# tanushreebanerjee/generative-detection

Measured on AMD Instinct MI355X. Metric: VAE train images/s (fwd+bwd+opt) at 256x256 z=16x16x16, higher is better.
Workload: dtype f32; 1 GPU; autoencoder_kl_16x16x16.yaml, 256x256 synthetic crops, B=32/GPU, rec+KL only (discriminator off, optimizer 0), fp32, VAE phase; global_batch=32, parallelism=dp1

## Files before the change

generative-detection_amd/build.py:

```python
import os
import subprocess
import sys
from concurrent.futures import ThreadPoolExecutor

HERE = os.path.dirname(os.path.abspath(__file__))
CSRC = os.path.join(HERE, "csrc")
OBJ_DIR = os.path.join(HERE, "build")
LIB_PATH = os.path.join(HERE, "libodvae_hip.so")
HIP_SOURCES = ["gemm_f32.hip", "gemm_f32_split.hip", "conv3x3_f32.hip", "conv3x3_wino_f32.hip", "conv3x3_wino4_f32.hip", "conv3x3_wgrad_f32.hip", "conv3x3_wgrad_wino_f32.hip", "groupnorm.hip", "elementwise.hip",
               "gan_f32.hip", "lpips_f32.hip", "patch_u8.hip", "pose_f32.hip", "linear_f32.hip",
               "conv_bf16.hip", "conv_wgrad_bf16.hip", "flash_attn_bf16.hip", "bf16_ops.hip",
               "flash_attn_f32.hip", "linattn_f32.hip", "anomaly.hip"]
CXX_SOURCES = ["runtime.cpp"]
HIPCC = os.environ.get("HIPCC", "/opt/rocm/bin/hipcc")
FLAGS = ["--offload-arch=gfx950", "-O3", "-fPIC", "-std=c++17", "-I", CSRC]
PER_FILE_FLAGS = {"flash_attn_bf16.hip": ["-fno-slp-vectorize"], "gemm_f32_split.hip": ["-fno-slp-vectorize"]}


def _stale(target, deps):
    if not os.path.exists(target):
        return True
    t = os.path.getmtime(target)
    return any(os.path.getmtime(d) > t for d in deps)


def _compile(src):
    obj = os.path.join(OBJ_DIR, os.path.basename(src) + ".o")
    deps = [src, os.path.join(CSRC, "common.h"), os.path.join(CSRC, "bf16_common.h"), os.path.join(CSRC, "gn_finalize.h"), os.path.join(CSRC, "dropout_mask.h"), os.path.join(CSRC, "gemm_f32_tile.h"), os.path.join(CSRC, "resample.h"), os.path.abspath(__file__)]
    if _stale(obj, deps):
        cmd = [HIPCC] + FLAGS + PER_FILE_FLAGS.get(os.path.basename(src), []) + ["-c", src, "-o", obj]
        r = subprocess.run(cmd, capture_output=True, text=True)
        if r.returncode != 0:
# ... 25 lines not shown
```

generative-detection_amd/csrc/gemm_f32.hip:

```cpp
#include "gemm_f32_tile.h"
#include <type_traits>

namespace {

using namespace gemm_tile;
constexpr int LDS_KC = BK + 4;
constexpr int LDS_RC = BM + 4;
constexpr int TILE_FLOATS = BM * LDS_KC;
template <int BKT> struct DmaGeom {
  static constexpr unsigned TILE_B = BM * BKT * 4;
  static constexpr unsigned STAGE_B = 2 * TILE_B;
  static constexpr unsigned LDS_B = 2 * STAGE_B;
  static constexpr int SLOTS = BKT / 4;
  static constexpr int PER_THREAD = BM * SLOTS / 256;
  static constexpr int ROW_SHIFT = BKT == 32 ? 3 : 2, SWZ_SHIFT = BKT == 32 ? 1 : 2, SWZ_MASK = SLOTS - 1;
};
__device__ __forceinline__ float lds_ld32(unsigned a) { return *(const __attribute__((address_space(3))) float*)(uintptr_t)a; }

template <bool KC>
struct TileFetch {
  __amdgpu_buffer_rsrc_t rsrc;
  unsigned voff[4];
  unsigned step_bytes;
  int kvalid;
// ... 360 lines not shown
  const unsigned DMA_LDS_B = lds_bytes;
  const hipError_t e = hipFuncSetAttribute(reinterpret_cast<const void*>(kern), hipFuncAttributeMaxDynamicSharedMemorySize, (int)DMA_LDS_B);
  if (e != hipSuccess) {
    odvae_set_error("gemm_f32: hipFuncSetAttribute failed: %s", hipGetErrorString(e));
    return ODVAE_ERR_HIP;
  }
  hipLaunchKernelGGL(kern, grid, dim3(256), DMA_LDS_B, st, p);
  return ODVAE_OK;
}

}

extern "C" {

int odvae_gemm_select_staging(int mode) {
  const int prev = g_dma_mode;
  g_dma_mode = mode < 0 ? -1 : (mode > 2 ? 2 : mode);
  return prev;
}

size_t odvae_gemm_f32_workspace_bytes(int M, int N, int K, int batch) {
  const int s = choose_splits(M, N, K, batch);
  return s > 1 ? (size_t)s * batch * M * N * sizeof(float) : 0;
}

static int gemm_f32_impl(int transA, int transB, int M, int N, int K, float alpha,
                         const float* A, int lda, int64_t strideA,
                         const float* B, int ldb, int64_t strideB,
                         float* C, int ldc, int64_t strideC,
                         const float* bias, const float* residual, int batch,
                         void* workspace, size_t workspace_bytes, void* stream);

int odvae_gemm_f32(int transA, int transB, int M, int N, int K, float alpha,
                   const float* A, int lda, int64_t strideA,
                   const float* B, int ldb, int64_t strideB,
                   float* C, int ldc, int64_t strideC,
                   const float* bias, const float* residual, int batch,
                   void* workspace, size_t workspace_bytes, void* stream) {
  return gemm_f32_impl(transA, transB, M, N, K, alpha, A, lda, strideA, B, ldb, strideB, C, ldc, strideC, bias, residual, batch,
                       workspace, workspace_bytes, stream);
}

int odvae_gemm_pred_f32(int transA, int transB, int M, int N, int K, float alpha,
                        const float* A, int lda, int64_t strideA,
                        const float* B, int ldb, int64_t strideB,
                        float* C, int ldc, int64_t strideC, int batch, const int* pred, void* stream) {
// ... 203 lines not shown
```

generative-detection_amd/csrc/gemm_f32_split.hip:

```cpp
#include "gemm_f32_tile.h"

namespace {

using namespace gemm_tile;

constexpr unsigned PLANE_B = BM * BK * 2;
constexpr unsigned OPER_B = 3 * PLANE_B;
constexpr unsigned OOB = 0x7FFFFFF0u;
constexpr int HI = 0, MID = 1, LO = 2;

__device__ __forceinline__ unsigned tile_byte(int row, int slot) {
  const int f = ((row >> 2) & 1) | ((((row >> 1) ^ (row >> 3)) & 1) << 1);
  return (unsigned)(row * 64 + ((slot ^ f) << 4));
}

__device__ __forceinline__ void store_unit(unsigned lds_oper, int row, int slot, const float (&x)[8]) {
  u32x4 pl[3];
  split8(x, pl);
  const unsigned a = lds_oper + tile_byte(row, slot);
#pragma unroll
  for (int q = 0; q < 3; ++q) lds_st128(a + q * PLANE_B, pl[q]);
}

template <bool KC>
// ... 43 lines not shown
        }
    } else {
#pragma unroll
      for (int i = 0; i < 2; ++i)
#pragma unroll
        for (int j = 0; j < 8; ++j) {
          const unsigned soff = (unsigned)__builtin_amdgcn_readfirstlane(k0 + 16 * i + j) * ld_bytes;
          unsigned vo = voff[0];
          if (tail && k0 + 8 * (tid >> 7) + 16 * i + j >= kvalid) vo = OOB;
          x[i][j] = __uint_as_float(__builtin_amdgcn_raw_buffer_load_b32(rsrc, vo, soff, 0));
        }
    }
  }
  __device__ __forceinline__ void store(unsigned lds_oper) const {
    const int tid = threadIdx.x;
#pragma unroll
    for (int i = 0; i < 2; ++i) {
      if (KC) store_unit(lds_oper, (tid + 256 * i) >> 2, tid & 3, x[i]);
      else    store_unit(lds_oper, tid & 127, (tid >> 7) + 2 * i, x[i]);
    }
  }
};

template <bool A_KC, bool B_KC, int EPI>
__global__ __launch_bounds__(256, 3) void gemm_f32_split_kernel(GemmParams p) {
  constexpr bool ROWNORM = EPI == EPI_ROWNORM, EXPB = EPI == EPI_EXPB, SMB = EPI == EPI_SMB;
  static_assert(!ROWNORM || A_KC, "the row sums are taken by the k-contiguous loader");
  static_assert(!(EXPB || SMB) || (A_KC && B_KC), "the T x T tails belong to the NT form");
  __shared__ __attribute__((aligned(16))) char smem[2 * OPER_B];
  const int tile_m = blockIdx.x % p.tiles_m, tile_n = blockIdx.x / p.tiles_m, batch = blockIdx.z;
  const int m0 = tile_m * BM, n0 = tile_n * BN;
  const float* A = p.A + batch * p.sA;
  const float* B = p.B + batch * p.sB;
  const int lane = threadIdx.x & 63, wave = threadIdx.x >> 6;
  const int wm = wave >> 1, wn = wave & 1, li = lane & 31, h = lane >> 5;

  TileOut out;
  out.init(p.M, p.N, p.ldc, m0, n0);

  f32x16 acc[2][2];
#pragma unroll
  for (int a = 0; a < 2; ++a)
#pragma unroll
    for (int b = 0; b < 2; ++b)
#pragma unroll
      for (int r = 0; r < 16; ++r) acc[a][b][r] = 0.f;

  const unsigned ldsA = lds_addr_of(smem), ldsB = ldsA + OPER_B;
  unsigned adrA[2], adrB[2];
#pragma unroll
  for (int kk = 0; kk < 2; ++kk) {
    adrA[kk] = ldsA + tile_byte(wm * 64 + li, 2 * kk + h);
    adrB[kk] = ldsB + tile_byte(wn * 64 + li, 2 * kk + h);
  }

  SplitLoader<A_KC> fa;
  SplitLoader<B_KC> fb;
  fa.init(A, p.lda, m0, p.M, p.K);
  fb.init(B, p.ldb, n0, p.N, p.K);
  float rowl[2] = {0.f, 0.f};
  auto stage = [&]() {
    if constexpr (ROWNORM) {
#pragma unroll
      for (int i = 0; i < 2; ++i)
        rowl[i] += ((fa.x[i][0] + fa.x[i][1]) + (fa.x[i][2] + fa.x[i][3])) + ((fa.x[i][4] + fa.x[i][5]) + (fa.x[i][6] + fa.x[i][7]));
    }
    fa.store(ldsA);
    fb.store(ldsB);
  };
  auto products = [&]() {
#pragma unroll
    for (int kk = 0; kk < 2; ++kk) {
      bf16x8 a[2][3], b[2][3];
#pragma unroll
      for (int t = 0; t < 2; ++t)
#pragma unroll
        for (int q = 0; q < 3; ++q) {
          a[t][q] = frag_from_u32x4(lds_ld128(adrA[kk] + t * 2048u + q * PLANE_B));
          b[t][q] = frag_from_u32x4(lds_ld128(adrB[kk] + t * 2048u + q * PLANE_B));
        }
      constexpr int ORDER[6][2] = {{LO, HI}, {HI, LO}, {MID, MID}, {MID, HI}, {HI, MID}, {HI, HI}};
#pragma unroll
// ... 67 lines not shown

namespace gemm_tile {

bool split_eligible(int staging_mode, int transB, int M, int N, int K, int batch, const float* bias, const float* residual) {
  return staging_mode == -1 && choose_splits(M, N, K, batch) == 1 && transB == 0 && K >= 1024 && !bias && !residual;
}

constexpr int SPLIT_TT_MIN_K = 64;
bool split_tt_eligible(int staging_mode, int M, int N, int K, int batch) {
  return staging_mode == -1 && (int64_t)ceil_div(M, BM) * ceil_div(N, BN) * batch >= 512 && K >= SPLIT_TT_MIN_K;
}

int launch_split(const GemmParams& p, int transA, int epi, int batch, hipStream_t st) {
  const dim3 grid(p.tiles_m * ceil_div(p.N, BN), 1, batch), block(256);
  if (epi == EPI_EXPB)          hipLaunchKernelGGL((gemm_f32_split_kernel<true, true, EPI_EXPB>), grid, block, 0, st, p);
  else if (epi == EPI_SMB)      hipLaunchKernelGGL((gemm_f32_split_kernel<true, true, EPI_SMB>), grid, block, 0, st, p);
  else if (epi == EPI_ROWNORM)  hipLaunchKernelGGL((gemm_f32_split_kernel<true, false, EPI_ROWNORM>), grid, block, 0, st, p);
  else if (!transA)             hipLaunchKernelGGL((gemm_f32_split_kernel<true, false, EPI_NONE>), grid, block, 0, st, p);
  else                          hipLaunchKernelGGL((gemm_f32_split_kernel<false, false, EPI_NONE>), grid, block, 0, st, p);
  ODVAE_LAUNCH_CHECK("gemm_f32 (bf16 split)");
  return ODVAE_OK;
}

}
```

generative-detection_amd/csrc/gemm_f32_tile.h:

```cpp
#pragma once
#include "bf16_common.h"

namespace gemm_tile {

constexpr int BM = 128, BN = 128, BK = 32;

struct GemmParams {
  const float* A; const float* B; float* C;
  const float* bias; const float* residual;
  float* partial;
  int M, N, K;
  int lda, ldb, ldc;
  int64_t sA, sB, sC;
  float alpha;
  int splits, k_per_split;
  int tiles_m;
  const float* rowsub; const float* emul; int64_t sRow;
  const float* rowmul;
  float* rowout; int* flag;
  const int* pred;
};
constexpr int EPI_NONE = 0, EPI_SMB = 1, EPI_EXPB = 2, EPI_ROWNORM = 3;

inline int choose_splits(int M, int N, int K, int batch) {
// ... 99 lines not shown
  }

#define GEMM_TILE_STORE_SMB(o, crsrc, ersrc, acc, alpha, rmv)                                                                            \
  {                                                                                                                                      \
    _Pragma("unroll") for (int mt_ = 0; mt_ < 2; ++mt_) {                                                                                \
      float pv_[2][16];                                                                                                                  \
      _Pragma("unroll") for (int r_ = 0; r_ < 16; ++r_) {                                                                                \
        const unsigned rb_ = (o).row_byte(mt_, r_);                                                                                      \
        _Pragma("unroll") for (int nt_ = 0; nt_ < 2; ++nt_)                                                                              \
          pv_[nt_][r_] = __uint_as_float(__builtin_amdgcn_raw_buffer_load_b32(ersrc, rb_ + (o).colbyte[nt_], 0, 0));                     \
      }                                                                                                                                  \
      _Pragma("unroll") for (int r_ = 0; r_ < 16; ++r_) {                                                                                \
        const unsigned rb_ = (o).row_byte(mt_, r_);                                                                                      \
        _Pragma("unroll") for (int nt_ = 0; nt_ < 2; ++nt_)                                                                              \
          __builtin_amdgcn_raw_buffer_store_b32(__float_as_uint((acc)[mt_][nt_][r_] * ((alpha) * (rmv)[mt_][r_]) * pv_[nt_][r_]), crsrc, \
                                                rb_ + (o).colbyte[nt_], 0, 0);                                                           \
      }                                                                                                                                  \
    }                                                                                                                                    \
  }

bool split_eligible(int staging_mode, int transB, int M, int N, int K, int batch, const float* bias, const float* residual);
bool split_tt_eligible(int staging_mode, int M, int N, int K, int batch);
int launch_split(const GemmParams& p, int transA, int epi, int batch, hipStream_t st);

}
```

generative-detection_amd/lib.py:

```python
import ctypes
import os
import re

import torch

_HERE = os.path.dirname(os.path.abspath(__file__))
LIB_PATH = os.path.join(_HERE, "libodvae_hip.so")
HEADER_PATH = os.path.join(os.path.dirname(_HERE), "include", "odvae_hip.h")

_c = ctypes
_P, _I, _L, _F, _Z = _c.c_void_p, _c.c_int, _c.c_int64, _c.c_float, _c.c_size_t
_D, _U64 = _c.c_double, _c.c_uint64

ABI_VERSION = 4

PROTOTYPES = {
    "odvae_last_error": (_c.c_char_p, []),
    "odvae_abi_version": (_I, []),
    "odvae_target_arch": (_c.c_char_p, []),
    "odvae_gemm_f32_workspace_bytes": (_Z, [_I, _I, _I, _I]),
    "odvae_gemm_select_staging": (_I, [_I]),
    "odvae_gemm_f32": (_I, [_I, _I, _I, _I, _I, _F, _P, _I, _L, _P, _I, _L, _P, _I, _L, _P, _P, _I, _P, _Z, _P]),
    "odvae_gemm_softmax_bwd_f32": (_I, [_I, _I, _I, _F, _P, _I, _L, _P, _I, _L, _P, _P, _L, _P, _I, _L, _I, _P]),
    "odvae_rowdot_f32": (_I, [_P, _P, _L, _I, _P, _P]),
    "odvae_attn_row_bound_f32": (_I, [_P, _I, _I, _I, _P, _P, _P, _P]),
    "odvae_gemm_exp_bound_f32": (_I, [_I, _I, _I, _F, _P, _I, _L, _P, _I, _L, _P, _L, _P, _I, _L, _I, _P]),
    "odvae_gemm_rownorm_f32": (_I, [_I, _I, _I, _P, _I, _L, _P, _I, _L, _P, _I, _L, _P, _L, _P, _I, _P]),
    "odvae_gemm_pred_f32": (_I, [_I, _I, _I, _I, _I, _F, _P, _I, _L, _P, _I, _L, _P, _I, _L, _I, _P, _P]),
    "odvae_softmax_rows_pred_f32": (_I, [_P, _P, _L, _I, _F, _P, _P, _P]),
    "odvae_rowdot_scale_f32": (_I, [_P, _P, _P, _L, _I, _P, _P, _P]),
    "odvae_gemm_softmax_bwd_scaled_f32": (_I, [_I, _I, _I, _F, _P, _I, _L, _P, _I, _L, _P, _P, _P, _L, _P, _I, _L, _I, _P]),
    "odvae_conv3x3_pack_reduce_pad": (_I, [_I]),
    "odvae_conv3x3_pack_out_pad": (_I, [_I]),
    "odvae_conv3x3_pack_floats": (_Z, [_I, _I]),
    "odvae_conv3x3_pack_f32": (_I, [_P, _I, _I, _P, _P, _P]),
    "odvae_conv3x3_up_pack_floats": (_Z, [_I, _I]),
    "odvae_conv3x3_pack_up_f32": (_I, [_P, _I, _I, _P, _P, _P]),
    "odvae_conv3x3_wino_reduce_pad": (_I, [_I]),
    "odvae_conv3x3_wino_out_pad": (_I, [_I]),
    "odvae_conv3x3_wino_pack_floats": (_Z, [_I, _I]),
    "odvae_conv3x3_pack_wino_f32": (_I, [_P, _I, _I, _P, _P, _P]),
    "odvae_conv3x3_wino_f32": (_I, [_P, _I, _I, _I, _I, _P, _I, _P, _P, _P, _I, _P]),
    "odvae_conv3x3_wino4_reduce_pad": (_I, [_I]),
    "odvae_conv3x3_wino4_out_pad": (_I, [_I]),
    "odvae_conv3x3_wino4_pack_floats": (_Z, [_I, _I]),
    "odvae_conv3x3_wino4_supported": (_I, [_I, _I, _I, _I]),
    "odvae_conv3x3_pack_wino4_f32": (_I, [_P, _I, _I, _P, _P, _P]),
    "odvae_conv3x3_pack_wino_batch": (_I, [_P, _I, _P]),
    "odvae_conv3x3_pack_wino4_batch": (_I, [_P, _I, _P]),
    "odvae_conv3x3_wino4_f32": (_I, [_P, _I, _I, _I, _I, _P, _I, _P, _P, _P, _I, _P]),
    "odvae_conv3x3_wino4_stats_chunks": (_I, [_I, _I]),
    "odvae_conv3x3_wino4_stats_f32": (_I, [_P, _I, _I, _I, _I, _P, _I, _P, _P, _P, _P, _I, _P]),
    "odvae_conv3x3_wino4_up_f32": (_I, [_P, _I, _I, _I, _I, _P, _I, _P, _P, _P, _P, _I, _P]),
    "odvae_conv3x3_wino4_pool_f32": (_I, [_P, _I, _I, _I, _I, _P, _I, _P, _P]),
# ... 245 lines not shown
```

generative-detection_amd/ops.py:

```python
import collections
import contextlib
import os
import weakref

import torch
from torch.autograd import Function

from . import lib as _lib

CL = torch.channels_last


def _L():
    return _lib.load()


BF16 = torch.bfloat16


def _cl(t, dtype=torch.float32):
    _lib.require_device(t, dtypes=(dtype,))
    if t.dim() != 4:
        raise ValueError("expected a 4-d NCHW tensor, got shape %s" % (tuple(t.shape),))
    n, c, h, w = t.shape
# ... 545 lines not shown
        if ctx.needs_input_grad[1]:
            dw2 = torch.empty(cout, cin, dtype=torch.float32, device=x.device)
            gemm(1, 0, cout, cin, m, 1.0, dy, cout, 0, x, cin, 0, dw2, cin, 0)
            dw = dw2.view(cout, cin, 1, 1)
        if ctx.has_bias and ctx.needs_input_grad[2]:
            db = _colsum(dy, m, cout)
        dres = dy if ctx.has_res and ctx.needs_input_grad[3] else None
        return dx, dw, db, dres


def conv1x1(x, weight, bias=None, residual=None, out_f32=False):
    if x.dtype == BF16:
        return _ConvB.apply(x, weight, bias, residual, 4, bool(out_f32))
    return _Conv1x1.apply(x, weight, bias, residual)


FUSED_SOFTMAX_BWD = os.environ.get("ODVAE_ATTN_UNFUSED", "0") != "1"


ATTN_FOLDED_SOFTMAX = os.environ.get("ODVAE_ATTN_FOLDED_SOFTMAX", "1") != "0"
_ATTN_LAST_FLAG = None


def _qkv_views(t, c):
    off = t.storage_offset()
    return tuple(t.as_strided((1,), (1,), off + i * c) for i in range(3))


class _Attention(Function):

    @staticmethod
    def forward(ctx, qkv):
        L = _L()
        qkv = _cl(qkv)
        n, c3, h, w = qkv.shape
        c = c3 // 3
        t = h * w
        scale = float(c) ** -0.5
        p = torch.empty(n, t, t, dtype=torch.float32, device=qkv.device)
        o = _new_cl(n, c, h, w, qkv)
        q, k, v = _qkv_views(qkv, c)
        sq = t * c3
        rinv = None
        if ATTN_FOLDED_SOFTMAX and L.odvae_gemm_f32_workspace_bytes(t, t, c, n) == 0 and L.odvae_gemm_f32_workspace_bytes(t, c, t, n) == 0:
            st = _lib.stream_ptr()
            bound = torch.empty(2, n * t, dtype=torch.float32, device=qkv.device)
            rinv = torch.empty(n * t, dtype=torch.float32, device=qkv.device)
            flag = torch.empty(1, dtype=torch.int32, device=qkv.device)
            _lib.check(L.odvae_attn_row_bound_f32(q.data_ptr(), n, t, c, bound.data_ptr(), bound[1].data_ptr(), flag.data_ptr(), st), "attn_row_bound")
            tag = KERNEL_EVENTS.begin(secondary=True)
            _lib.check(L.odvae_gemm_exp_bound_f32(t, t, c, scale, q.data_ptr(), c3, sq, k.data_ptr(), c3, sq, bound.data_ptr(), t,
                                                  p.data_ptr(), t, t * t, n, st), "gemm_exp_bound")
            KERNEL_EVENTS.end("gemm_f32", 2.0 * t * t * c * n, tag, 4.0 * n * (2 * t * c + t * t))
            tag = KERNEL_EVENTS.begin(secondary=True)
            _lib.check(L.odvae_gemm_rownorm_f32(t, c, t, p.data_ptr(), t, t * t, v.data_ptr(), c3, sq, o.data_ptr(), c, t * c,
                                                rinv.data_ptr(), t, flag.data_ptr(), n, st), "gemm_rownorm")
            KERNEL_EVENTS.end("gemm_f32", 2.0 * t * t * c * n, tag, 4.0 * n * (2 * t * c + t * t))
            _lib.check(L.odvae_gemm_pred_f32(0, 1, t, t, c, 1.0, q.data_ptr(), c3, sq, k.data_ptr(), c3, sq, p.data_ptr(), t, t * t, n,
                                             flag.data_ptr(), st), "gemm_pred(QK^T)")
            _lib.check(L.odvae_softmax_rows_pred_f32(p.data_ptr(), p.data_ptr(), n * t, t, scale, flag.data_ptr(), rinv.data_ptr(), st), "softmax_rows_pred")
            _lib.check(L.odvae_gemm_pred_f32(0, 0, t, c, t, 1.0, p.data_ptr(), t, t * t, v.data_ptr(), c3, sq, o.data_ptr(), c, t * c, n,
                                             flag.data_ptr(), st), "gemm_pred(PV)")
            global _ATTN_LAST_FLAG
            _ATTN_LAST_FLAG = flag
        else:
            gemm(0, 1, t, t, c, 1.0, q, c3, sq, k, c3, sq, p, t, t * t, batch=n)
            _lib.check(L.odvae_softmax_rows_f32(p.data_ptr(), p.data_ptr(), n * t, t, scale, _lib.stream_ptr()), "softmax_rows")
            gemm(0, 0, t, c, t, 1.0, p, t, t * t, v, c3, sq, o, c, t * c, batch=n)
        ctx.folded = rinv is not None
        if rinv is not None:
            ctx.save_for_backward(qkv, p, o, rinv)
        else:
            ctx.save_for_backward(qkv, p, o)
        return o

    @staticmethod
    def backward(ctx, do):
        L = _L()
        if ctx.folded:
            qkv, p, o, rinv = ctx.saved_tensors
        else:
            (qkv, p, o), rinv = ctx.saved_tensors, None
        do = _cl(do)
        n, c3, h, w = qkv.shape
        c = c3 // 3
        t = h * w
        scale = float(c) ** -0.5
        sq = t * c3
        q, k, v = _qkv_views(qkv, c)
        dqkv = _new_cl(n, c3, h, w, qkv)
        dq, dk, dv = _qkv_views(dqkv, c)
        if rinv is not None:
            drow = torch.empty(n * t, dtype=torch.float32, device=p.device)
            dos = torch.empty_like(do)
            _lib.check(L.odvae_rowdot_scale_f32(do.data_ptr(), o.data_ptr(), rinv.data_ptr(), n * t, c, drow.data_ptr(), dos.data_ptr(),
                                                _lib.stream_ptr()), "rowdot_scale")
            gemm(1, 0, t, c, t, 1.0, p, t, t * t, dos, c, t * c, dv, c3, sq, batch=n)
            del dos
            dp = torch.empty_like(p)
            tag = KERNEL_EVENTS.begin(secondary=True)
            _lib.check(L.odvae_gemm_softmax_bwd_scaled_f32(t, t, c, scale, do.data_ptr(), c, t * c, v.data_ptr(), c3, sq, p.data_ptr(),
                                                           drow.data_ptr(), rinv.data_ptr(), t, dp.data_ptr(), t, t * t, n, _lib.stream_ptr()),
                       "gemm_softmax_bwd_scaled")
            KERNEL_EVENTS.end("gemm_f32", 2.0 * t * t * c * n, tag, 4.0 * n * (2 * t * c + 2 * t * t))
            gemm(0, 0, t, c, t, 1.0, dp, t, t * t, k, c3, sq, dq, c3, sq, batch=n)
            gemm(1, 0, t, c, t, 1.0, dp, t, t * t, q, c3, sq, dk, c3, sq, batch=n)
            return dqkv
        gemm(1, 0, t, c, t, 1.0, p, t, t * t, do, c, t * c, dv, c3, sq, batch=n)
        dp = torch.empty_like(p)
        if FUSED_SOFTMAX_BWD:
            drow = torch.empty(n * t, dtype=torch.float32, device=p.device)
            _lib.check(L.odvae_rowdot_f32(do.data_ptr(), o.data_ptr(), n * t, c, drow.data_ptr(), _lib.stream_ptr()), "rowdot")
            tag = KERNEL_EVENTS.begin(secondary=True)
            _lib.check(L.odvae_gemm_softmax_bwd_f32(t, t, c, scale, do.data_ptr(), c, t * c, v.data_ptr(), c3, sq, p.data_ptr(),
                                                    drow.data_ptr(), t, dp.data_ptr(), t, t * t, n, _lib.stream_ptr()),
                       "gemm_softmax_bwd")
            KERNEL_EVENTS.end("gemm_f32", 2.0 * t * t * c * n, tag, 4.0 * n * (2 * t * c + 2 * t * t))
        else:
            gemm(0, 1, t, t, c, 1.0, do, c, t * c, v, c3, sq, dp, t, t * t, batch=n)
            _lib.check(L.odvae_softmax_rows_bwd_f32(p.data_ptr(), dp.data_ptr(), dp.data_ptr(), n * t, t, scale,
                                                    _lib.stream_ptr()), "softmax_rows_bwd")
        gemm(0, 0, t, c, t, 1.0, dp, t, t * t, k, c3, sq, dq, c3, sq, batch=n)
        gemm(1, 0, t, c, t, 1.0, dp, t, t * t, q, c3, sq, dk, c3, sq, batch=n)
        return dqkv


ATTN_SCORE_BUDGET = int(float(os.environ.get("ODVAE_ATTN_SCORE_BUDGET_GB", "4")) * 2 ** 30)


# ... 1302 lines not shown
```

include/odvae_hip.h:

```cpp
#ifndef ODVAE_HIP_H
#define ODVAE_HIP_H

#include <stddef.h>
#include <stdint.h>

#ifdef __cplusplus
extern "C" {
#endif

#define ODVAE_ABI_VERSION 4
#define ODVAE_OK 0
#define ODVAE_ERR_ARG 1
#define ODVAE_ERR_WORKSPACE 2
#define ODVAE_ERR_HIP 3

const char* odvae_last_error(void);
int odvae_abi_version(void);
const char* odvae_target_arch(void);

size_t odvae_gemm_f32_workspace_bytes(int M, int N, int K, int batch);
int odvae_gemm_select_staging(int mode);
int odvae_gemm_f32(int transA, int transB, int M, int N, int K, float alpha,
                   const float* A, int lda, int64_t strideA,
                   const float* B, int ldb, int64_t strideB,
// ... 85 lines not shown
int odvae_groupnorm_fused_timeouts(void);
int odvae_device_health(int* gn_timeouts, int* attn_fallbacks, int inject_gn_timeouts, int inject_attn_fallbacks);
int odvae_attn_softmax_fallbacks(int add);
int odvae_groupnorm_recentred(int add);

int odvae_softmax_rows_f32(const float* x, float* y, int64_t rows, int cols, float scale, void* stream);
int odvae_softmax_rows_bwd_f32(const float* p, const float* dp, float* ds, int64_t rows, int cols, float scale, void* stream);
int odvae_rowdot_f32(const float* a, const float* b, int64_t rows, int cols, float* out, void* stream);
int odvae_gemm_softmax_bwd_f32(int M, int N, int K, float alpha, const float* A, int lda, int64_t strideA,
                               const float* B, int ldb, int64_t strideB, const float* P, const float* rowdot,
                               int64_t strideRow, float* dS, int ldc, int64_t strideC, int batch, void* stream);
int odvae_attn_row_bound_f32(const float* qkv, int N, int T, int C, float* bound, float* nk_scratch, int* flag, void* stream);
int odvae_gemm_exp_bound_f32(int M, int N, int K, float alpha, const float* A, int lda, int64_t strideA, const float* B, int ldb, int64_t strideB,
                             const float* rowbound, int64_t strideRow, float* E, int ldc, int64_t strideC, int batch, void* stream);
int odvae_gemm_rownorm_f32(int M, int N, int K, const float* A, int lda, int64_t strideA, const float* B, int ldb, int64_t strideB,
                           float* C, int ldc, int64_t strideC, float* rinv, int64_t strideRow, int* flag, int batch, void* stream);
int odvae_gemm_pred_f32(int transA, int transB, int M, int N, int K, float alpha, const float* A, int lda, int64_t strideA,
                        const float* B, int ldb, int64_t strideB, float* C, int ldc, int64_t strideC, int batch, const int* pred, void* stream);
int odvae_softmax_rows_pred_f32(const float* x, float* y, int64_t rows, int cols, float scale, const int* pred, float* ones, void* stream);
int odvae_rowdot_scale_f32(const float* a, const float* b, const float* row_scale, int64_t rows, int cols, float* out, float* a_scaled, void* stream);
int odvae_gemm_softmax_bwd_scaled_f32(int M, int N, int K, float alpha, const float* A, int lda, int64_t strideA,
                                      const float* B, int ldb, int64_t strideB, const float* E, const float* rowdot, const float* rinv,
                                      int64_t strideRow, float* dS, int ldc, int64_t strideC, int batch, void* stream);
int odvae_upsample2x_bwd_f32(const float* du, float* dx, int N, int H, int W, int C, void* stream);
int odvae_avgpool2x2_f32(const float* x, float* y, int N, int H, int W, int C, float* gn_partial, int gn_groups, int chunks, void* stream);
int odvae_avgpool2x2_bwd_f32(const float* dy, float* dx, int N, int H, int W, int C, void* stream);
int odvae_upsample2x_f32(const float* x, float* u, int N, int H, int W, int C, float* gn_partial, int gn_groups, int chunks, void* stream);
int odvae_tanh_f32(const float* x, float* y, int64_t n, void* stream);
int odvae_tanh_bwd_f32(const float* y, const float* dy, float* dx, int64_t n, void* stream);
int odvae_rescale_minmax_f32(const float* x_nchw, float* y_nhwc, int N, int C, int HW, float* minmax_out,
                             void* workspace, size_t workspace_bytes, void* stream);
int odvae_gaussian_sample_f32(const float* moments, const float* eps, float* z, int N, int HW, int Cz, void* stream);
int odvae_gaussian_kl_f32(const float* moments, float* kl, int N, int HW, int Cz, void* stream);
int odvae_gaussian_bwd_f32(const float* moments, const float* eps, const float* dz, const float* dkl,
                           float* dmoments, int N, int HW, int Cz, void* stream);
int odvae_l1_masked_sum_f32(const float* x, const float* xr, const float* mask, float* out, int N, int HW, int C,
                            void* workspace, size_t workspace_bytes, void* stream);
int odvae_l1_masked_bwd_f32(const float* x, const float* xr, const float* mask, const float* g, float* dxr,
                            int N, int HW, int C, void* stream);
size_t odvae_colsum_workspace_bytes(int64_t rows, int C);
int odvae_colsum_f32(const float* x, int64_t rows, int C, float* out, void* workspace, size_t workspace_bytes, void* stream);
int odvae_grad_norm_f32(const float* g, int64_t n, float max_norm, float* out, void* workspace, size_t workspace_bytes, void* stream);
int odvae_adam_step_f32(float* p, const float* g, float* m, float* v, int64_t n, float lr, float beta1, float beta2,
                        float eps, int step, const float* clip, void* stream);
int odvae_grad_accumulate_segments_per_launch(void);
int odvae_grad_accumulate_f32(float* arena, int64_t arena_numel, const int64_t* dst_off, const float* const* src, const int64_t* numel,
// ... 122 lines not shown
```

Measured before the change: 154.9 images/s.

## Pre-split attention GEMM operands into bf16 planes once and reuse across GEMMs

Adds a presplit kernel that converts f32 operands (Q, K, V, dO, optionally row-scaled) into three bf16 planes stored in global memory. The split-bf16 GEMM kernel gets a plane loader that reads these planes with b128 buffer loads instead of splitting f32 values per tile. Attention forward and backward use this path when the shapes are eligible. Splitting happens once per operand instead of once per tile per GEMM, at the cost of extra plane buffers and extra presplit launches.

```diff
diff --git a/generative-detection_amd/build.py b/generative-detection_amd/build.py
--- a/generative-detection_amd/build.py
+++ b/generative-detection_amd/build.py
@@ -7,7 +7,7 @@
 CSRC = os.path.join(HERE, "csrc")
 OBJ_DIR = os.path.join(HERE, "build")
 LIB_PATH = os.path.join(HERE, "libodvae_hip.so")
-HIP_SOURCES = ["gemm_f32.hip", "gemm_f32_split.hip", "conv3x3_f32.hip", "conv3x3_wino_f32.hip", "conv3x3_wino4_f32.hip", "conv3x3_wgrad_f32.hip", "conv3x3_wgrad_wino_f32.hip", "groupnorm.hip", "elementwise.hip",
+HIP_SOURCES = ["gemm_f32.hip", "gemm_f32_split.hip", "gemm_presplit.hip", "conv3x3_f32.hip", "conv3x3_wino_f32.hip", "conv3x3_wino4_f32.hip", "conv3x3_wgrad_f32.hip", "conv3x3_wgrad_wino_f32.hip", "groupnorm.hip", "elementwise.hip",
                "gan_f32.hip", "lpips_f32.hip", "patch_u8.hip", "pose_f32.hip", "linear_f32.hip",
                "conv_bf16.hip", "conv_wgrad_bf16.hip", "flash_attn_bf16.hip", "bf16_ops.hip",
                "flash_attn_f32.hip", "linattn_f32.hip", "anomaly.hip"]
diff --git a/generative-detection_amd/csrc/gemm_f32.hip b/generative-detection_amd/csrc/gemm_f32.hip
--- a/generative-detection_amd/csrc/gemm_f32.hip
+++ b/generative-detection_amd/csrc/gemm_f32.hip
@@ -406,6 +406,10 @@
 size_t odvae_gemm_f32_workspace_bytes(int M, int N, int K, int batch) {
   const int s = choose_splits(M, N, K, batch);
   return s > 1 ? (size_t)s * batch * M * N * sizeof(float) : 0;
+}
+
+int odvae_gemm_split_eligible(int nt, int M, int N, int K, int batch) {
+  return nt ? split_tt_eligible(g_dma_mode, M, N, K, batch) : split_eligible(g_dma_mode, 0, M, N, K, batch, nullptr, nullptr);
 }
 
 static int gemm_f32_impl(int transA, int transB, int M, int N, int K, float alpha,
diff --git a/generative-detection_amd/csrc/gemm_f32_split.hip b/generative-detection_amd/csrc/gemm_f32_split.hip
--- a/generative-detection_amd/csrc/gemm_f32_split.hip
+++ b/generative-detection_amd/csrc/gemm_f32_split.hip
@@ -1,4 +1,5 @@
 #include "gemm_f32_tile.h"
+#include <type_traits>
 
 namespace {
 
@@ -89,16 +90,60 @@
   }
 };
 
-template <bool A_KC, bool B_KC, int EPI>
+struct PlaneLoader {
+  __amdgpu_buffer_rsrc_t rsrc;
+  unsigned voff[2];
+  unsigned plane_bytes;
+  int kvalid;
+  u32x4 v[2][3];
+
+  __device__ __forceinline__ void init(const bf16_t* G, int ld, int64_t plane_stride, int row0, int nrows, int K) {
+    const int tid = threadIdx.x;
+    kvalid = K;
+    plane_bytes = (unsigned)plane_stride * 2u;
+    const int rows = min(BM, nrows - row0);
+    const int64_t bytes = (2 * plane_stride + (int64_t)(rows - 1) * ld + ((K + 7) & ~7)) * 2;
+    rsrc = __builtin_amdgcn_make_buffer_rsrc(const_cast<bf16_t*>(G) + (int64_t)row0 * ld, 0, (int)(bytes < 0x7FFFFFF0ll ? bytes : 0x7FFFFFF0ll), 0x00020000);
+#pragma unroll
+    for (int i = 0; i < 2; ++i) {
+      const int u = tid + 256 * i;
+      voff[i] = (u >> 2) < rows ? (unsigned)(((u >> 2) * ld + 8 * (u & 3)) * 2) : OOB;
+    }
+  }
+  template <bool TAIL>
+  __device__ __forceinline__ void load(int k0) {
+    const int tid = threadIdx.x;
+    const bool tail = TAIL && k0 + BK > kvalid;
+    const unsigned soff = (unsigned)__builtin_amdgcn_readfirstlane(k0) * 2u;
+#pragma unroll
+    for (int i = 0; i < 2; ++i) {
+      unsigned vo = voff[i];
+      if (tail && k0 + 8 * (tid & 3) >= kvalid) vo = OOB;
+#pragma unroll
+      for (int q = 0; q < 3; ++q) v[i][q] = __builtin_amdgcn_raw_buffer_load_b128(rsrc, vo, soff + (unsigned)q * plane_bytes, 0);
+    }
+  }
+  __device__ __forceinline__ void store(unsigned lds_oper) const {
+    const int tid = threadIdx.x;
+#pragma unroll
+    for (int i = 0; i < 2; ++i) {
+      const unsigned a = lds_oper + tile_byte((tid + 256 * i) >> 2, tid & 3);
+#pragma unroll
+      for (int q = 0; q < 3; ++q) lds_st128(a + q * PLANE_B, v[i][q]);
+    }
+  }
+};
+
+template <bool A_KC, bool B_KC, int EPI, bool A_PL = false, bool B_PL = false>
 __global__ __launch_bounds__(256, 3) void gemm_f32_split_kernel(GemmParams p) {
   constexpr bool ROWNORM = EPI == EPI_ROWNORM, EXPB = EPI == EPI_EXPB, SMB = EPI == EPI_SMB;
-  static_assert(!ROWNORM || A_KC, "the row sums are taken by the k-contiguous loader");
+  static_assert(!ROWNORM || (A_KC && !A_PL), "the row sums are taken by the k-contiguous loader, from the unsplit values");
   static_assert(!(EXPB || SMB) || (A_KC && B_KC), "the T x T tails belong to the NT form");
   __shared__ __attribute__((aligned(16))) char smem[2 * OPER_B];
   const int tile_m = blockIdx.x % p.tiles_m, tile_n = blockIdx.x / p.tiles_m, batch = blockIdx.z;
   const int m0 = tile_m * BM, n0 = tile_n * BN;
-  const float* A = p.A + batch * p.sA;
-  const float* B = p.B + batch * p.sB;
+  [[maybe_unused]] const float* A = p.A + batch * p.sA;
+  [[maybe_unused]] const float* B = p.B + batch * p.sB;
   const int lane = threadIdx.x & 63, wave = threadIdx.x >> 6;
   const int wm = wave >> 1, wn = wave & 1, li = lane & 31, h = lane >> 5;
 
@@ -121,10 +166,12 @@
     adrB[kk] = ldsB + tile_byte(wn * 64 + li, 2 * kk + h);
   }
 
-  SplitLoader<A_KC> fa;
-  SplitLoader<B_KC> fb;
-  fa.init(A, p.lda, m0, p.M, p.K);
-  fb.init(B, p.ldb, n0, p.N, p.K);
+  std::conditional_t<A_PL, PlaneLoader, SplitLoader<A_KC>> fa;
+  std::conditional_t<B_PL, PlaneLoader, SplitLoader<B_KC>> fb;
+  if constexpr (A_PL) fa.init(reinterpret_cast<const bf16_t*>(p.A) + 3 * batch * p.sA, p.lda, p.sA, m0, p.M, p.K);
+  else                fa.init(A, p.lda, m0, p.M, p.K);
+  if constexpr (B_PL) fb.init(reinterpret_cast<const bf16_t*>(p.B) + 3 * batch * p.sB, p.ldb, p.sB, n0, p.N, p.K);
+  else                fb.init(B, p.ldb, n0, p.N, p.K);
   float rowl[2] = {0.f, 0.f};
   auto stage = [&]() {
     if constexpr (ROWNORM) {
@@ -238,4 +285,15 @@
   return ODVAE_OK;
 }
 
-}
+int launch_split_planes(const GemmParams& p, int transA, int epi, int batch, hipStream_t st) {
+  const dim3 grid(p.tiles_m * ceil_div(p.N, BN), 1, batch), block(256);
+  if (epi == EPI_EXPB)          hipLaunchKernelGGL((gemm_f32_split_kernel<true, true, EPI_EXPB, true, true>), grid, block, 0, st, p);
+  else if (epi == EPI_SMB)      hipLaunchKernelGGL((gemm_f32_split_kernel<true, true, EPI_SMB, true, true>), grid, block, 0, st, p);
+  else if (epi == EPI_ROWNORM)  hipLaunchKernelGGL((gemm_f32_split_kernel<true, false, EPI_ROWNORM, false, true>), grid, block, 0, st, p);
+  else if (!transA)             hipLaunchKernelGGL((gemm_f32_split_kernel<true, false, EPI_NONE, false, true>), grid, block, 0, st, p);
+  else                          hipLaunchKernelGGL((gemm_f32_split_kernel<false, false, EPI_NONE, false, true>), grid, block, 0, st, p);
+  ODVAE_LAUNCH_CHECK("gemm_f32 (bf16 split, pre-split operands)");
+  return ODVAE_OK;
+}
+
+}
diff --git a/generative-detection_amd/csrc/gemm_f32_tile.h b/generative-detection_amd/csrc/gemm_f32_tile.h
--- a/generative-detection_amd/csrc/gemm_f32_tile.h
+++ b/generative-detection_amd/csrc/gemm_f32_tile.h
@@ -145,5 +145,6 @@
 bool split_eligible(int staging_mode, int transB, int M, int N, int K, int batch, const float* bias, const float* residual);
 bool split_tt_eligible(int staging_mode, int M, int N, int K, int batch);
 int launch_split(const GemmParams& p, int transA, int epi, int batch, hipStream_t st);
+int launch_split_planes(const GemmParams& p, int transA, int epi, int batch, hipStream_t st);
 
 }
diff --git a/generative-detection_amd/csrc/gemm_presplit.hip b/generative-detection_amd/csrc/gemm_presplit.hip
--- /dev/null
+++ b/generative-detection_amd/csrc/gemm_presplit.hip
@@ -0,0 +1,176 @@
+#include "gemm_f32_tile.h"
+
+namespace {
+
+using namespace gemm_tile;
+
+__device__ __forceinline__ f32x4 ld_f32x4(const float* p) { return *reinterpret_cast<const f32x4*>(p); }
+
+__global__ __launch_bounds__(256) void presplit_channel_kernel(const float* __restrict__ x, int ld, int64_t sx, const float* __restrict__ rs,
+                                                               int T, int C, int Cp, bf16_t* __restrict__ out) {
+  const int upr = Cp >> 3, n = blockIdx.y;
+  const int64_t units = (int64_t)T * upr;
+  for (int64_t u = (int64_t)blockIdx.x * 256 + threadIdx.x; u < units; u += (int64_t)gridDim.x * 256) {
+    const int tok = (int)(u / upr), c0 = (int)(u - (int64_t)tok * upr) * 8;
+    const float* px = x + n * sx + (int64_t)tok * ld + c0;
+    const f32x4 a = ld_f32x4(px);
+    const f32x4 b = c0 + 4 < C ? ld_f32x4(px + 4) : f32x4{0.f, 0.f, 0.f, 0.f};
+    float v[8] = {a.x, a.y, a.z, a.w, b.x, b.y, b.z, b.w};
+    if (rs) {
+      const float r = rs[(int64_t)n * T + tok];
+#pragma unroll
+      for (int j = 0; j < 8; ++j) v[j] = __fmul_rn(v[j], r);
+    }
+    u32x4 pl[3];
+    split8(v, pl);
+#pragma unroll
+    for (int q = 0; q < 3; ++q)
+      *reinterpret_cast<u32x4*>(out + (((int64_t)n * 3 + q) * T + tok) * Cp + c0) = pl[q];
+  }
+}
+
+constexpr int PT = 64, PC = 64;
+__global__ __launch_bounds__(256) void presplit_token_kernel(const float* __restrict__ x, int ld, int64_t sx, const float* __restrict__ rs,
+                                                             int T, int C, int Tp, bf16_t* __restrict__ out) {
+  __shared__ float tile[PT][PC + 1];
+  const int t0 = blockIdx.x * PT, c0 = blockIdx.y * PC, n = blockIdx.z, tid = threadIdx.x;
+#pragma unroll
+  for (int i = 0; i < 4; ++i) {
+    const int f = tid + 256 * i, tok = f >> 4, c4 = (f & 15) * 4;
+    f32x4 a = {0.f, 0.f, 0.f, 0.f};
+    if (t0 + tok < T && c0 + c4 < C) {
+      a = ld_f32x4(x + n * sx + (int64_t)(t0 + tok) * ld + c0 + c4);
+      if (rs) {
+        const float r = rs[(int64_t)n * T + t0 + tok];
+        a.x = __fmul_rn(a.x, r); a.y = __fmul_rn(a.y, r); a.z = __fmul_rn(a.z, r); a.w = __fmul_rn(a.w, r);
+      }
+    }
+    tile[tok][c4] = a.x; tile[tok][c4 + 1] = a.y; tile[tok][c4 + 2] = a.z; tile[tok][c4 + 3] = a.w;
+  }
+  __syncthreads();
+#pragma unroll
+  for (int i = 0; i < 2; ++i) {
+    const int u = tid + 256 * i, tu = u & 7, ch = u >> 3;
+    float v[8];
+#pragma unroll
+    for (int j = 0; j < 8; ++j) v[j] = tile[tu * 8 + j][ch];
+    u32x4 pl[3];
+    split8(v, pl);
+    if (c0 + ch < C && t0 + tu * 8 < Tp) {
+#pragma unroll
+      for (int q = 0; q < 3; ++q)
+        *reinterpret_cast<u32x4*>(out + (((int64_t)n * 3 + q) * C + c0 + ch) * Tp + t0 + tu * 8) = pl[q];
+    }
+  }
+}
+
+inline int round8(int v) { return (v + 7) & ~7; }
+
+int check_planes(const char* who, const void* P, int ld, int64_t ps, int64_t stride, int rows, int K) {
+  ODVAE_CHECK_ARG(P && ((uintptr_t)P & 15) == 0, "%s: planes must be non-null and 16-byte aligned", who);
+  ODVAE_CHECK_ARG(ld % 8 == 0 && ps % 8 == 0 && stride % 8 == 0, "%s: plane ld / plane stride / batch stride must be multiples of 8 (ld=%d)", who, ld);
+  ODVAE_CHECK_ARG(ld >= round8(K), "%s: plane ld %d < K rounded up to 8 (K=%d)", who, ld, K);
+  ODVAE_CHECK_ARG(ps >= (int64_t)rows * ld, "%s: plane stride %lld < rows * ld", who, (long long)ps);
+  ODVAE_CHECK_ARG(stride == 3 * ps, "%s: the three planes of an image are adjacent: batch stride %lld != 3 * plane stride %lld", who,
+                  (long long)stride, (long long)ps);
+  ODVAE_CHECK_ARG((2 * ps + (int64_t)BM * ld) * 2 < 0x7FFFFFF0ll, "%s: one block's window over the three planes exceeds 2 GiB", who);
+  return ODVAE_OK;
+}
+
+void base_params(GemmParams& p, int M, int N, int K, float alpha, float* C, int ldc, int64_t strideC) {
+  p.C = C; p.bias = nullptr; p.residual = nullptr; p.partial = nullptr;
+  p.M = M; p.N = N; p.K = K; p.ldc = ldc; p.sC = strideC; p.alpha = alpha;
+  p.splits = 1; p.k_per_split = ceil_div(K, BK) * BK; p.tiles_m = ceil_div(M, BM);
+  p.rowsub = nullptr; p.emul = nullptr; p.sRow = 0; p.rowmul = nullptr; p.rowout = nullptr; p.flag = nullptr; p.pred = nullptr;
+}
+
+int tdeep_impl(const char* who, int transA, int epi, GemmParams& p, const float* A, int lda, int64_t strideA,
+               const void* Bp, int ldbp, int64_t psB, int64_t strideBp, int batch, void* stream) {
+  ODVAE_CHECK_ARG(p.M > 0 && p.N > 0 && p.K > 0 && batch > 0 && batch <= 65535, "%s: bad shape M=%d N=%d K=%d batch=%d", who, p.M, p.N, p.K, batch);
+  ODVAE_CHECK_ARG(A && p.C, "%s: null operand", who);
+  ODVAE_CHECK_ARG((int64_t)BM * p.ldc * 4 < 0x7FFFFFF0ll, "%s: ldc %d too large for 32-bit tile offsets", who, p.ldc);
+  ODVAE_CHECK_ARG(lda % 4 == 0 && strideA % 4 == 0 && ((uintptr_t)A & 15) == 0, "%s: lda / strideA must be multiples of 4 floats, A 16-byte aligned", who);
+  if (!transA) ODVAE_CHECK_ARG(p.K % 4 == 0, "%s: a k-contiguous A needs K %% 4 == 0 (K=%d)", who, p.K);
+  ODVAE_CHECK_ARG((transA ? (int64_t)p.k_per_split * lda : (int64_t)BM * lda) * 4 < 0x7FFFFFF0ll, "%s: one block's window of A exceeds 2 GiB", who);
+  const int rc = check_planes(who, Bp, ldbp, psB, strideBp, p.N, p.K);
+  if (rc != ODVAE_OK) return rc;
+  p.A = A; p.lda = lda; p.sA = strideA;
+  p.B = static_cast<const float*>(Bp); p.ldb = ldbp; p.sB = psB;
+  return launch_split_planes(p, transA, epi, batch, static_cast<hipStream_t>(stream));
+}
+
+int nt_impl(const char* who, int epi, GemmParams& p, const void* Ap, int ldap, int64_t psA, int64_t strideAp,
+            const void* Bp, int ldbp, int64_t psB, int64_t strideBp, int batch, void* stream) {
+  ODVAE_CHECK_ARG(p.M > 0 && p.N > 0 && p.K > 0 && batch > 0 && batch <= 65535, "%s: bad shape M=%d N=%d K=%d batch=%d", who, p.M, p.N, p.K, batch);
+  ODVAE_CHECK_ARG(p.C && p.rowsub, "%s: null operand", who);
+  ODVAE_CHECK_ARG((int64_t)BM * p.ldc * 4 < 0x7FFFFFF0ll, "%s: ldc %d too large for 32-bit tile offsets", who, p.ldc);
+  int rc = check_planes(who, Ap, ldap, psA, strideAp, p.M, p.K);
+  if (rc != ODVAE_OK) return rc;
+  rc = check_planes(who, Bp, ldbp, psB, strideBp, p.N, p.K);
+  if (rc != ODVAE_OK) return rc;
+  p.A = static_cast<const float*>(Ap); p.lda = ldap; p.sA = psA;
+  p.B = static_cast<const float*>(Bp); p.ldb = ldbp; p.sB = psB;
+  return launch_split_planes(p, 0, epi, batch, static_cast<hipStream_t>(stream));
+}
+
+}
+
+extern "C" {
+
+int odvae_split_planes_f32(const float* x, int ld, int64_t stride, const float* row_scale, int batch, int T, int C, int token_contiguous,
+                           void* planes, void* stream) {
+  ODVAE_CHECK_ARG(x && planes && batch > 0 && batch <= 65535 && T > 0 && C > 0, "split_planes: bad arguments (batch=%d T=%d C=%d)", batch, T, C);
+  ODVAE_CHECK_ARG(C % 4 == 0 && ld % 4 == 0 && ld >= C && stride % 4 == 0, "split_planes: C, ld and the batch stride must be multiples of 4 floats, ld >= C");
+  ODVAE_CHECK_ARG(((uintptr_t)x & 15) == 0 && ((uintptr_t)planes & 15) == 0, "split_planes: x and planes must be 16-byte aligned");
+  hipStream_t st = static_cast<hipStream_t>(stream);
+  bf16_t* out = static_cast<bf16_t*>(planes);
+  if (token_contiguous) {
+    ODVAE_CHECK_ARG(ceil_div(C, PC) <= 65535, "split_planes: C %d too large", C);
+    hipLaunchKernelGGL(presplit_token_kernel, dim3(ceil_div(T, PT), ceil_div(C, PC), batch), dim3(256), 0, st, x, ld, stride, row_scale, T, C, round8(T), out);
+  } else {
+    const int Cp = round8(C);
+    const int64_t blocks = ceil_div64((int64_t)T * (Cp >> 3), 256);
+    hipLaunchKernelGGL(presplit_channel_kernel, dim3((unsigned)std::min<int64_t>(blocks, 65536), batch), dim3(256), 0, st, x, ld, stride, row_scale, T, C, Cp, out);
+  }
+  ODVAE_LAUNCH_CHECK("split_planes");
+  return ODVAE_OK;
+}
+
+int odvae_gemm_presplit_f32(int transA, int M, int N, int K, float alpha, const float* A, int lda, int64_t strideA,
+                            const void* Bp, int ldbp, int64_t planeB, int64_t strideBp, float* C, int ldc, int64_t strideC, int batch, void* stream) {
+  GemmParams p;
+  base_params(p, M, N, K, alpha, C, ldc, strideC);
+  if (transA) ODVAE_CHECK_ARG(M % 4 == 0, "gemm_presplit: transA needs M %% 4 == 0 (M=%d)", M);
+  return tdeep_impl("gemm_presplit", transA != 0, EPI_NONE, p, A, lda, strideA, Bp, ldbp, planeB, strideBp, batch, stream);
+}
+
+int odvae_gemm_rownorm_presplit_f32(int M, int N, int K, const float* A, int lda, int64_t strideA, const void* Bp, int ldbp, int64_t planeB,
+                                    int64_t strideBp, float* C, int ldc, int64_t strideC, float* rinv, int64_t strideRow, int* flag, int batch,
+                                    void* stream) {
+  ODVAE_CHECK_ARG(rinv, "gemm_rownorm_presplit: null operand");
+  GemmParams p;
+  base_params(p, M, N, K, 1.f, C, ldc, strideC);
+  p.sRow = strideRow; p.rowout = rinv; p.flag = flag;
+  return tdeep_impl("gemm_rownorm_presplit", 0, EPI_ROWNORM, p, A, lda, strideA, Bp, ldbp, planeB, strideBp, batch, stream);
+}
+
+int odvae_gemm_exp_bound_presplit_f32(int M, int N, int K, float alpha, const void* Ap, int ldap, int64_t planeA, int64_t strideAp,
+                                      const void* Bp, int ldbp, int64_t planeB, int64_t strideBp, const float* rowbound, int64_t strideRow,
+                                      float* E, int ldc, int64_t strideC, int batch, void* stream) {
+  GemmParams p;
+  base_params(p, M, N, K, alpha, E, ldc, strideC);
+  p.rowsub = rowbound; p.sRow = strideRow;
+  return nt_impl("gemm_exp_bound_presplit", EPI_EXPB, p, Ap, ldap, planeA, strideAp, Bp, ldbp, planeB, strideBp, batch, stream);
+}
+
+int odvae_gemm_softmax_bwd_presplit_f32(int M, int N, int K, float alpha, const void* Ap, int ldap, int64_t planeA, int64_t strideAp,
+                                        const void* Bp, int ldbp, int64_t planeB, int64_t strideBp, const float* P, const float* rowdot,
+                                        const float* rinv, int64_t strideRow, float* dS, int ldc, int64_t strideC, int batch, void* stream) {
+  ODVAE_CHECK_ARG(P, "gemm_softmax_bwd_presplit: null operand");
+  GemmParams p;
+  base_params(p, M, N, K, alpha, dS, ldc, strideC);
+  p.rowsub = rowdot; p.emul = P; p.sRow = strideRow; p.rowmul = rinv;
+  return nt_impl("gemm_softmax_bwd_presplit", EPI_SMB, p, Ap, ldap, planeA, strideAp, Bp, ldbp, planeB, strideBp, batch, stream);
+}
+
+}
diff --git a/generative-detection_amd/lib.py b/generative-detection_amd/lib.py
--- a/generative-detection_amd/lib.py
+++ b/generative-detection_amd/lib.py
@@ -30,6 +30,12 @@
     "odvae_softmax_rows_pred_f32": (_I, [_P, _P, _L, _I, _F, _P, _P, _P]),
     "odvae_rowdot_scale_f32": (_I, [_P, _P, _P, _L, _I, _P, _P, _P]),
     "odvae_gemm_softmax_bwd_scaled_f32": (_I, [_I, _I, _I, _F, _P, _I, _L, _P, _I, _L, _P, _P, _P, _L, _P, _I, _L, _I, _P]),
+    "odvae_gemm_split_eligible": (_I, [_I, _I, _I, _I, _I]),
+    "odvae_split_planes_f32": (_I, [_P, _I, _L, _P, _I, _I, _I, _I, _P, _P]),
+    "odvae_gemm_presplit_f32": (_I, [_I, _I, _I, _I, _F, _P, _I, _L, _P, _I, _L, _L, _P, _I, _L, _I, _P]),
+    "odvae_gemm_rownorm_presplit_f32": (_I, [_I, _I, _I, _P, _I, _L, _P, _I, _L, _L, _P, _I, _L, _P, _L, _P, _I, _P]),
+    "odvae_gemm_exp_bound_presplit_f32": (_I, [_I, _I, _I, _F, _P, _I, _L, _L, _P, _I, _L, _L, _P, _L, _P, _I, _L, _I, _P]),
+    "odvae_gemm_softmax_bwd_presplit_f32": (_I, [_I, _I, _I, _F, _P, _I, _L, _L, _P, _I, _L, _L, _P, _P, _P, _L, _P, _I, _L, _I, _P]),
     "odvae_conv3x3_pack_reduce_pad": (_I, [_I]),
     "odvae_conv3x3_pack_out_pad": (_I, [_I]),
     "odvae_conv3x3_pack_floats": (_Z, [_I, _I]),
diff --git a/generative-detection_amd/ops.py b/generative-detection_amd/ops.py
--- a/generative-detection_amd/ops.py
+++ b/generative-detection_amd/ops.py
@@ -591,6 +591,40 @@
 _ATTN_LAST_FLAG = None
 
 
+_ATTN_PRESPLIT_ENV = os.environ.get("ODVAE_ATTN_PRESPLIT", "0")
+ATTN_PRESPLIT = {"0": False, "1": True}.get(_ATTN_PRESPLIT_ENV, _ATTN_PRESPLIT_ENV)
+
+
+def _presplit_forms(L, n, t, c):
+    if not ATTN_PRESPLIT or c % 8 != 0:
+        return ()
+    if not (L.odvae_gemm_split_eligible(1, t, t, c, n) and L.odvae_gemm_split_eligible(0, t, c, t, n)):
+        return ()
+    return ("nt", "td") if ATTN_PRESPLIT is True else tuple(f for f in ("nt", "td") if f in str(ATTN_PRESPLIT).split(","))
+
+
+class _Planes:
+
+    def __init__(self, x, ld, stride, n, t, c, token, ref, row_scale=None):
+        self.token, self.t, self.c = token, t, c
+        self.ld = (t + 7) // 8 * 8 if token else (c + 7) // 8 * 8
+        self.plane = (c if token else t) * self.ld
+        self.buf = torch.empty(n * 3 * self.plane, dtype=torch.bfloat16, device=ref.device)
+        _lib.check(_L().odvae_split_planes_f32(x.data_ptr(), ld, stride, _lib.ptr(row_scale), n, t, c, int(token), self.buf.data_ptr(),
+                                               _lib.stream_ptr()), "split_planes")
+
+    def part(self, i=0, w=None):
+        off = 0 if w is None else (i * w * self.ld if self.token else i * w)
+        return self.buf.data_ptr() + 2 * off, self.ld, self.plane, 3 * self.plane
+
+
+def _gemm_presplit(ta, m, nn, k, a, lda, sa, bp, c, ldc, sc, batch):
+    tag = KERNEL_EVENTS.begin(secondary=True)
+    _lib.check(_L().odvae_gemm_presplit_f32(int(ta), m, nn, k, 1.0, a.data_ptr(), lda, sa, bp[0], bp[1], bp[2], bp[3], c.data_ptr(), ldc, sc,
+                                            batch, _lib.stream_ptr()), "gemm_presplit")
+    KERNEL_EVENTS.end("gemm_f32", 2.0 * m * nn * k * batch, tag, 4.0 * batch * (m * k + k * nn + m * nn))
+
+
 def _qkv_views(t, c):
     off = t.storage_offset()
     return tuple(t.as_strided((1,), (1,), off + i * c) for i in range(3))
@@ -617,14 +651,33 @@
             rinv = torch.empty(n * t, dtype=torch.float32, device=qkv.device)
             flag = torch.empty(1, dtype=torch.int32, device=qkv.device)
             _lib.check(L.odvae_attn_row_bound_f32(q.data_ptr(), n, t, c, bound.data_ptr(), bound[1].data_ptr(), flag.data_ptr(), st), "attn_row_bound")
-            tag = KERNEL_EVENTS.begin(secondary=True)
-            _lib.check(L.odvae_gemm_exp_bound_f32(t, t, c, scale, q.data_ptr(), c3, sq, k.data_ptr(), c3, sq, bound.data_ptr(), t,
-                                                  p.data_ptr(), t, t * t, n, st), "gemm_exp_bound")
-            KERNEL_EVENTS.end("gemm_f32", 2.0 * t * t * c * n, tag, 4.0 * n * (2 * t * c + t * t))
-            tag = KERNEL_EVENTS.begin(secondary=True)
-            _lib.check(L.odvae_gemm_rownorm_f32(t, c, t, p.data_ptr(), t, t * t, v.data_ptr(), c3, sq, o.data_ptr(), c, t * c,
-                                                rinv.data_ptr(), t, flag.data_ptr(), n, st), "gemm_rownorm")
-            KERNEL_EVENTS.end("gemm_f32", 2.0 * t * t * c * n, tag, 4.0 * n * (2 * t * c + t * t))
+            forms = _presplit_forms(L, n, t, c)
+            if "nt" in forms:
+                qk = _Planes(q, c3, sq, n, t, 2 * c, False, qkv)
+                qp, kp = qk.part(0, c), qk.part(1, c)
+                tag = KERNEL_EVENTS.begin(secondary=True)
+                _lib.check(L.odvae_gemm_exp_bound_presplit_f32(t, t, c, scale, qp[0], qp[1], qp[2], qp[3], kp[0], kp[1], kp[2], kp[3],
+                                                               bound.data_ptr(), t, p.data_ptr(), t, t * t, n, st), "gemm_exp_bound_presplit")
+                KERNEL_EVENTS.end("gemm_f32", 2.0 * t * t * c * n, tag, 4.0 * n * (2 * t * c + t * t))
+                del qk
+            else:
+                tag = KERNEL_EVENTS.begin(secondary=True)
+                _lib.check(L.odvae_gemm_exp_bound_f32(t, t, c, scale, q.data_ptr(), c3, sq, k.data_ptr(), c3, sq, bound.data_ptr(), t,
+                                                      p.data_ptr(), t, t * t, n, st), "gemm_exp_bound")
+                KERNEL_EVENTS.end("gemm_f32", 2.0 * t * t * c * n, tag, 4.0 * n * (2 * t * c + t * t))
+            if "td" in forms:
+                vp = _Planes(v, c3, sq, n, t, c, True, qkv)
+                vb = vp.part()
+                tag = KERNEL_EVENTS.begin(secondary=True)
+                _lib.check(L.odvae_gemm_rownorm_presplit_f32(t, c, t, p.data_ptr(), t, t * t, vb[0], vb[1], vb[2], vb[3], o.data_ptr(), c, t * c,
+                                                             rinv.data_ptr(), t, flag.data_ptr(), n, st), "gemm_rownorm_presplit")
+                KERNEL_EVENTS.end("gemm_f32", 2.0 * t * t * c * n, tag, 4.0 * n * (2 * t * c + t * t))
+                del vp
+            else:
+                tag = KERNEL_EVENTS.begin(secondary=True)
+                _lib.check(L.odvae_gemm_rownorm_f32(t, c, t, p.data_ptr(), t, t * t, v.data_ptr(), c3, sq, o.data_ptr(), c, t * c,
+                                                    rinv.data_ptr(), t, flag.data_ptr(), n, st), "gemm_rownorm")
+                KERNEL_EVENTS.end("gemm_f32", 2.0 * t * t * c * n, tag, 4.0 * n * (2 * t * c + t * t))
             _lib.check(L.odvae_gemm_pred_f32(0, 1, t, t, c, 1.0, q.data_ptr(), c3, sq, k.data_ptr(), c3, sq, p.data_ptr(), t, t * t, n,
                                              flag.data_ptr(), st), "gemm_pred(QK^T)")
             _lib.check(L.odvae_softmax_rows_pred_f32(p.data_ptr(), p.data_ptr(), n * t, t, scale, flag.data_ptr(), rinv.data_ptr(), st), "softmax_rows_pred")
@@ -661,19 +714,43 @@
         dq, dk, dv = _qkv_views(dqkv, c)
         if rinv is not None:
             drow = torch.empty(n * t, dtype=torch.float32, device=p.device)
-            dos = torch.empty_like(do)
-            _lib.check(L.odvae_rowdot_scale_f32(do.data_ptr(), o.data_ptr(), rinv.data_ptr(), n * t, c, drow.data_ptr(), dos.data_ptr(),
-                                                _lib.stream_ptr()), "rowdot_scale")
-            gemm(1, 0, t, c, t, 1.0, p, t, t * t, dos, c, t * c, dv, c3, sq, batch=n)
-            del dos
+            forms = _presplit_forms(L, n, t, c)
+            if "td" in forms:
+                _lib.check(L.odvae_rowdot_f32(do.data_ptr(), o.data_ptr(), n * t, c, drow.data_ptr(), _lib.stream_ptr()), "rowdot")
+                dosp = _Planes(do, c, t * c, n, t, c, True, do, row_scale=rinv)
+                _gemm_presplit(1, t, c, t, p, t, t * t, dosp.part(), dv, c3, sq, n)
+                del dosp
+            else:
+                dos = torch.empty_like(do)
+                _lib.check(L.odvae_rowdot_scale_f32(do.data_ptr(), o.data_ptr(), rinv.data_ptr(), n * t, c, drow.data_ptr(), dos.data_ptr(),
+                                                    _lib.stream_ptr()), "rowdot_scale")
+                gemm(1, 0, t, c, t, 1.0, p, t, t * t, dos, c, t * c, dv, c3, sq, batch=n)
+                del dos
             dp = torch.empty_like(p)
-            tag = KERNEL_EVENTS.begin(secondary=True)
-            _lib.check(L.odvae_gemm_softmax_bwd_scaled_f32(t, t, c, scale, do.data_ptr(), c, t * c, v.data_ptr(), c3, sq, p.data_ptr(),
-                                                           drow.data_ptr(), rinv.data_ptr(), t, dp.data_ptr(), t, t * t, n, _lib.stream_ptr()),
-                       "gemm_softmax_bwd_scaled")
-            KERNEL_EVENTS.end("gemm_f32", 2.0 * t * t * c * n, tag, 4.0 * n * (2 * t * c + 2 * t * t))
-            gemm(0, 0, t, c, t, 1.0, dp, t, t * t, k, c3, sq, dq, c3, sq, batch=n)
-            gemm(1, 0, t, c, t, 1.0, dp, t, t * t, q, c3, sq, dk, c3, sq, batch=n)
+            if "nt" in forms:
+                dop = _Planes(do, c, t * c, n, t, c, False, do)
+                vcp = _Planes(v, c3, sq, n, t, c, False, do)
+                ap, bp = dop.part(), vcp.part()
+                tag = KERNEL_EVENTS.begin(secondary=True)
+                _lib.check(L.odvae_gemm_softmax_bwd_presplit_f32(t, t, c, scale, ap[0], ap[1], ap[2], ap[3], bp[0], bp[1], bp[2], bp[3],
+                                                                 p.data_ptr(), drow.data_ptr(), rinv.data_ptr(), t, dp.data_ptr(), t, t * t, n,
+                                                                 _lib.stream_ptr()), "gemm_softmax_bwd_presplit")
+                KERNEL_EVENTS.end("gemm_f32", 2.0 * t * t * c * n, tag, 4.0 * n * (2 * t * c + 2 * t * t))
+                del dop, vcp
+            else:
+                tag = KERNEL_EVENTS.begin(secondary=True)
+                _lib.check(L.odvae_gemm_softmax_bwd_scaled_f32(t, t, c, scale, do.data_ptr(), c, t * c, v.data_ptr(), c3, sq, p.data_ptr(),
+                                                               drow.data_ptr(), rinv.data_ptr(), t, dp.data_ptr(), t, t * t, n, _lib.stream_ptr()),
+                           "gemm_softmax_bwd_scaled")
+                KERNEL_EVENTS.end("gemm_f32", 2.0 * t * t * c * n, tag, 4.0 * n * (2 * t * c + 2 * t * t))
+            if "td" in forms:
+                qkt = _Planes(q, c3, sq, n, t, 2 * c, True, do)
+                _gemm_presplit(0, t, c, t, dp, t, t * t, qkt.part(1, c), dq, c3, sq, n)
+                _gemm_presplit(1, t, c, t, dp, t, t * t, qkt.part(0, c), dk, c3, sq, n)
+                del qkt
+            else:
+                gemm(0, 0, t, c, t, 1.0, dp, t, t * t, k, c3, sq, dq, c3, sq, batch=n)
+                gemm(1, 0, t, c, t, 1.0, dp, t, t * t, q, c3, sq, dk, c3, sq, batch=n)
             return dqkv
         gemm(1, 0, t, c, t, 1.0, p, t, t * t, do, c, t * c, dv, c3, sq, batch=n)
         dp = torch.empty_like(p)
diff --git a/include/odvae_hip.h b/include/odvae_hip.h
--- a/include/odvae_hip.h
+++ b/include/odvae_hip.h
@@ -131,6 +131,20 @@
 int odvae_gemm_softmax_bwd_scaled_f32(int M, int N, int K, float alpha, const float* A, int lda, int64_t strideA,
                                       const float* B, int ldb, int64_t strideB, const float* E, const float* rowdot, const float* rinv,
                                       int64_t strideRow, float* dS, int ldc, int64_t strideC, int batch, void* stream);
+int odvae_gemm_split_eligible(int nt, int M, int N, int K, int batch);
+int odvae_split_planes_f32(const float* x, int ld, int64_t stride, const float* row_scale, int batch, int T, int C, int token_contiguous,
+                           void* planes, void* stream);
+int odvae_gemm_presplit_f32(int transA, int M, int N, int K, float alpha, const float* A, int lda, int64_t strideA,
+                            const void* Bp, int ldbp, int64_t planeB, int64_t strideBp, float* C, int ldc, int64_t strideC, int batch, void* stream);
+int odvae_gemm_rownorm_presplit_f32(int M, int N, int K, const float* A, int lda, int64_t strideA, const void* Bp, int ldbp, int64_t planeB,
+                                    int64_t strideBp, float* C, int ldc, int64_t strideC, float* rinv, int64_t strideRow, int* flag, int batch,
+                                    void* stream);
+int odvae_gemm_exp_bound_presplit_f32(int M, int N, int K, float alpha, const void* Ap, int ldap, int64_t planeA, int64_t strideAp,
+                                      const void* Bp, int ldbp, int64_t planeB, int64_t strideBp, const float* rowbound, int64_t strideRow,
+                                      float* E, int ldc, int64_t strideC, int batch, void* stream);
+int odvae_gemm_softmax_bwd_presplit_f32(int M, int N, int K, float alpha, const void* Ap, int ldap, int64_t planeA, int64_t strideAp,
+                                        const void* Bp, int ldbp, int64_t planeB, int64_t strideBp, const float* P, const float* rowdot,
+                                        const float* rinv, int64_t strideRow, float* dS, int ldc, int64_t strideC, int batch, void* stream);
 int odvae_upsample2x_bwd_f32(const float* du, float* dx, int N, int H, int W, int C, void* stream);
 int odvae_avgpool2x2_f32(const float* x, float* y, int N, int H, int W, int C, float* gn_partial, int gn_groups, int chunks, void* stream);
 int odvae_avgpool2x2_bwd_f32(const float* dy, float* dx, int N, int H, int W, int C, void* stream);
```

Result: no change. 155.0 images/s, median of 2 (+0.1%).
